# zprodev/zlib.es

Hardware: AMD Instinct MI355X
Metric: GiB/s deflate+inflate round trip, 64 MiB buffers (uncompressed bytes / wall), bit-exact vs reference (higher is better)
Workload: dtype u8; 1 GPU; random64: 1 x 64 MiB xorshift buffer(s) per GPU (seed 12345+index), deflate then inflate, HBM-resident; bytes_per_buffer=67108864, compressed_bytes=67176156, parallelism=independent buffers, one per GPU

## Files before the change

### zlib.es_amd/csrc/zes_inflate_par.hip

```cpp
#include "zes_common.h"
#include "zes_kernels.h"
#include "zes_chain.h"

#define PL_ROOT 10u
#define PD_ROOT 9u
#define F_EOB 1u
#define F_FAIL 2u
#define F_VOID 4u
#define F_HIST 8u

#define RES_W 4096u
#define P4_SPARSE_DEP_MAX 32u
#define P4_SPARSE_MAX 1024u
#ifndef RES_REPS
#define RES_REPS 4u
#endif
#define PAR_CHUNK (ZES_BLK - 3u * RES_W)
#define PAR_DIST_OFF (PAR_CHUNK + 64u)
#define PAR_MAX_OUT (1u << 27)
#define STAGE_DW ((ZES_BLK + ZES_BLK / 8) / 4)
struct ParSmem {
  uint8_t out[ZES_BLK];
  uint32_t bitmap[ZES_BLK / 32];
  uint32_t lut_l[1u << PL_ROOT];
  uint32_t lut_d[1u << PD_ROOT];
  uint8_t len_l[1u << PL_ROOT];
  uint8_t len_d[1u << PD_ROOT];
  uint16_t syms_l[288];
  uint16_t syms_d[32];
  uint32_t first_l[16], first_d[16];
  uint16_t cnt_l[16], cnt_d[16], offs_l[16], offs_d[16];
  uint8_t lens[352];
  uint8_t cl_lut[128];
  uint32_t wave_sum[PAR_WAVES];
  uint8_t wtab[PAR_WAVES][48];
  uint8_t gtab[PAR_WAVES][4][48];
  uint8_t wentry[PAR_WAVES];
  uint32_t hdr_end, status, tail_entry, bfinal, tail_bytes, tail_end;
  uint32_t h_hlit, h_total, h_wbase, h_off, h_k, h_prev, h_done;
  uint32_t res_flag[3];
  uint32_t res_lastw[RES_W / 32];
  uint32_t res_strad[4];
  uint32_t f8lo, f8n, f8off;
  uint32_t sp_n;
};

static_assert(offsetof(ParSmem, cl_lut) - offsetof(ParSmem, lut_l) >= RES_W * 2u, "P4's distance array lies over the decode tables");
static_assert(RES_W % PAR_THREADS == 0 && RES_W % 8u == 0, "P4 lane mapping");

__device__ __forceinline__ static uint32_t entry_l(uint32_t sym, uint32_t len) {
  if (sym < 256u) return len | (sym << 16);
  if (sym == 256u) return len | (1u << 8);
  if (sym < 286u) return len | ((uint32_t)kLenXbits[sym - 257u] << 4) | (2u << 8) | ((uint32_t)kLenBase[sym - 257u] << 16);
  return len | (3u << 8);
}
__device__ __forceinline__ static uint32_t entry_d(uint32_t sym, uint32_t len) {
  if (sym < 30u) return len | ((uint32_t)kDistXbits[sym] << 4) | (2u << 8) | ((uint32_t)kDistBase[sym] << 16);
  return len | (3u << 8);
}

struct BitSrc {
  const uint32_t* g32;
  uint32_t lastdw;
  const uint32_t* s32;
  uint32_t s_first;
  uint32_t s_count;
};
template <bool LDS>
__device__ __forceinline__ static uint32_t src_ldw(const BitSrc& s, uint32_t idx) {
  if (LDS) {
    const uint32_t k = idx - s.s_first;
    return k < s.s_count ? s.s32[k ^ ((k >> 5) & 31u)] : 0u;
  }
  return s.g32[idx < s.lastdw ? idx : s.lastdw];
}

struct LaneBits {
  uint64_t bb;
  uint32_t nb;
  uint32_t pos;
  uint32_t pre;
};
template <bool LDS>
__device__ __forceinline__ static void lb_seek(LaneBits& b, const BitSrc& s, uint32_t bit) {
  const uint32_t i = bit >> 5, sh = bit & 31u;
  const uint64_t w = (uint64_t)src_ldw<LDS>(s, i) | ((uint64_t)src_ldw<LDS>(s, i + 1) << 32);
  b.bb = w >> sh;
  b.nb = 64u - sh;
  b.pos = bit;
  b.pre = LDS ? 0u : src_ldw<LDS>(s, i + 2);
}
template <bool LDS>
__device__ __forceinline__ static void lb_refill(LaneBits& b, const BitSrc& s) {
  if (b.nb <= 32u) {
    if (LDS) {
      b.bb |= (uint64_t)src_ldw<LDS>(s, (b.pos + b.nb) >> 5) << b.nb;
      b.nb += 32u;
    } else {
      b.bb |= (uint64_t)b.pre << b.nb;
      b.nb += 32u;
      b.pre = src_ldw<LDS>(s, (b.pos + b.nb) >> 5);
    }
  }
}
__device__ __forceinline__ static uint32_t lb_take(LaneBits& b, uint32_t k) {
  const uint32_t v = (uint32_t)b.bb & ((1u << k) - 1u);
  b.bb >>= k;
  b.nb -= k;
  b.pos += k;
  return v;
}

struct Lit8 {
  uint32_t lo, n, off;
};
__device__ __forceinline__ static uint32_t lead_lit8(uint32_t w, const Lit8& f) {
  const uint32_t r = __brev(w);
  const bool a = ((r >> 24) - f.lo) < f.n, b = (((r >> 16) & 255u) - f.lo) < f.n, c = (((r >> 8) & 255u) - f.lo) < f.n,
             d = ((r & 255u) - f.lo) < f.n;
  uint32_t n = d ? 4u : 3u;
  n = c ? n : 2u;
  n = b ? n : 1u;
  n = a ? n : 0u;
  return n;
}

struct SegTab {
  uint64_t a, b, c, d, e, f, g, h;
};
__device__ __forceinline__ static uint32_t tab_get(const SegTab& t, uint32_t o) {
  const uint32_t wi = o >> 3;
  uint64_t a = t.a, b = t.b, c = t.c, d = t.d, e = t.e, f = t.f, g = t.g, h = t.h;
  asm("" : "+v"(a), "+v"(b), "+v"(c), "+v"(d));
  asm("" : "+v"(e), "+v"(f), "+v"(g), "+v"(h));
  uint64_t x = a;
  x = (wi == 1u) ? b : x;
  x = (wi == 2u) ? c : x;
  x = (wi == 3u) ? d : x;
  x = (wi == 4u) ? e : x;
  x = (wi == 5u) ? f : x;
  x = (wi == 6u) ? g : x;
  x = (wi == 7u) ? h : x;
  return (uint32_t)(x >> ((o & 7u) * 8u)) & 0xffu;
}
__device__ __forceinline__ static void tab_set(SegTab& t, uint32_t o, uint32_t code) {
  const uint32_t wi = o >> 3;
  const uint64_t v = (uint64_t)code << ((o & 7u) * 8u);
  t.a |= (wi == 0u) ? v : 0ull;
  t.b |= (wi == 1u) ? v : 0ull;
  t.c |= (wi == 2u) ? v : 0ull;
  t.d |= (wi == 3u) ? v : 0ull;
  t.e |= (wi == 4u) ? v : 0ull;
  t.f |= (wi == 5u) ? v : 0ull;
  t.g |= (wi == 6u) ? v : 0ull;
  t.h |= (wi == 7u) ? v : 0ull;
}
__device__ __forceinline__ static void tab_put(SegTab& t, uint32_t o, uint32_t code, bool doit) {
  const uint32_t wi = o >> 3, sh = (o & 7u) * 8u;
  const uint64_t m = doit ? (0xffull << sh) : 0ull, v = doit ? ((uint64_t)code << sh) : 0ull;
  t.a = (wi == 0u) ? ((t.a & ~m) | v) : t.a;
  t.b = (wi == 1u) ? ((t.b & ~m) | v) : t.b;
  t.c = (wi == 2u) ? ((t.c & ~m) | v) : t.c;
  t.d = (wi == 3u) ? ((t.d & ~m) | v) : t.d;
  t.e = (wi == 4u) ? ((t.e & ~m) | v) : t.e;
  t.f = (wi == 5u) ? ((t.f & ~m) | v) : t.f;
  t.g = (wi == 6u) ? ((t.g & ~m) | v) : t.g;
  t.h = (wi == 7u) ? ((t.h & ~m) | v) : t.h;
}
__device__ __forceinline__ static uint64_t tab_nzmask(const SegTab& t) {
  auto nz8 = [](uint64_t w) -> uint64_t {
    const uint64_t k7 = 0x7f7f7f7f7f7f7f7full;
    const uint64_t y = (((w & k7) + k7) | w) & ~k7;
    return ((y >> 7) * 0x0102040810204080ull) >> 56;
  };
  return nz8(t.a) | (nz8(t.b) << 8) | (nz8(t.c) << 16) | (nz8(t.d) << 24) | (nz8(t.e) << 32) | (nz8(t.f) << 40) | (nz8(t.g) << 48) | (nz8(t.h) << 56);
}
__device__ __forceinline__ static uint64_t bcast64(uint64_t v, uint32_t srclane) {
  const uint32_t lo = (uint32_t)__builtin_amdgcn_readlane((int)(uint32_t)v, (int)srclane);
  const uint32_t hi = (uint32_t)__builtin_amdgcn_readlane((int)(uint32_t)(v >> 32), (int)srclane);
  return (uint64_t)lo | ((uint64_t)hi << 32);
}
__device__ __forceinline__ static SegTab tab_bcast(const SegTab& t, uint32_t srclane) {
  SegTab r;
  r.a = bcast64(t.a, srclane);
  r.b = bcast64(t.b, srclane);
  r.c = bcast64(t.c, srclane);
  r.d = bcast64(t.d, srclane);
  r.e = bcast64(t.e, srclane);
  r.f = bcast64(t.f, srclane);
  r.g = bcast64(t.g, srclane);
  r.h = bcast64(t.h, srclane);
  return r;
}

__device__ __forceinline__ static int slow_sym(const LaneBits& b, uint32_t root, const uint16_t* syms, const uint32_t* first,
                                               const uint16_t* cnt, const uint16_t* offs, uint32_t* len_out) {
  uint32_t code = __brev((uint32_t)b.bb & ((1u << root) - 1u)) >> (32u - root);
  for (uint32_t len = root + 1; len <= 15u; len++) {
    code = (code << 1) | (uint32_t)((b.bb >> (len - 1)) & 1u);
    const uint32_t f = first[len];
    const uint32_t rel = code - f;
    if (code >= f && rel < cnt[len]) {
      *len_out = len;
      return (int)syms[offs[len] + rel];
    }
  }
  return -1;
}

#define T_LIT 0u
#define T_EOB 1u
#define T_MATCH 2u
#define T_FAIL 3u
#define C_EOB 62u
#define C_FAIL 63u
#define C_NONE 255u

template <bool LDS>
__device__ __forceinline__ static uint32_t tok_step(ParSmem& S, LaneBits& b, const BitSrc& src, uint32_t& val, uint32_t& len,
                                                    uint32_t& dist) {
  lb_refill<LDS>(b, src);
  uint32_t e = S.lut_l[(uint32_t)b.bb & ((1u << PL_ROOT) - 1u)];
  if ((e & 15u) == 0u) {
    uint32_t l2 = 0;
    const int sy = slow_sym(b, PL_ROOT, S.syms_l, S.first_l, S.cnt_l, S.offs_l, &l2);
    if (sy < 0) return T_FAIL;
    e = entry_l((uint32_t)sy, l2);
  }
  lb_take(b, e & 15u);
  const uint32_t kind = (e >> 8) & 3u;
  if (kind == 0u) {
    val = e >> 16;
    return T_LIT;
  }
  if (kind == 1u) return T_EOB;
  if (kind == 3u) return T_FAIL;
  lb_refill<LDS>(b, src);
  len = (e >> 16) + lb_take(b, (e >> 4) & 15u);
  lb_refill<LDS>(b, src);
  uint32_t ed = S.lut_d[(uint32_t)b.bb & ((1u << PD_ROOT) - 1u)];
  if ((ed & 15u) == 0u) {
    uint32_t l2 = 0;
    const int sy = slow_sym(b, PD_ROOT, S.syms_d, S.first_d, S.cnt_d, S.offs_d, &l2);
    if (sy < 0) return T_FAIL;
    ed = entry_d((uint32_t)sy, l2);
  }
  lb_take(b, ed & 15u);
  if (((ed >> 8) & 3u) != 2u) return T_FAIL;
  lb_refill<LDS>(b, src);
  dist = (ed >> 16) + lb_take(b, (ed >> 4) & 15u);
  return T_MATCH;
}

__device__ __forceinline__ static uint32_t lut_l_entry(ParSmem& S, uint32_t bits) {
  uint32_t e = S.lut_l[bits & ((1u << PL_ROOT) - 1u)];
  if ((e & 15u) == 0u) {
    LaneBits t;
    t.bb = bits;
    uint32_t l2 = 0;
    const int sy = slow_sym(t, PL_ROOT, S.syms_l, S.first_l, S.cnt_l, S.offs_l, &l2);
    e = sy < 0 ? 0u : entry_l((uint32_t)sy, l2);
  }
  return e;
}
__device__ __forceinline__ static uint32_t lut_d_entry(ParSmem& S, uint32_t bits) {
  uint32_t e = S.lut_d[bits & ((1u << PD_ROOT) - 1u)];
  if ((e & 15u) == 0u) {
    LaneBits t;
    t.bb = bits;
    uint32_t l2 = 0;
    const int sy = slow_sym(t, PD_ROOT, S.syms_d, S.first_d, S.cnt_d, S.offs_d, &l2);
    e = sy < 0 ? 0u : entry_d((uint32_t)sy, l2);
  }
  return e;
}

__device__ __forceinline__ static void lb_refill_bf(LaneBits& b, const BitSrc& s) {
  const bool need = b.nb <= 32u;
  const uint32_t k = ((b.pos + b.nb) >> 5) - s.s_first;
  const bool in = k < s.s_count;
  const uint32_t kk = in ? k : 0u;
  uint32_t w = s.s32[kk ^ ((kk >> 5) & 31u)];
  w = in ? w : 0u;
  const uint32_t sh = need ? b.nb : 0u;
  const uint64_t add = (uint64_t)w << sh;
  b.bb |= need ? add : 0ull;
  b.nb += need ? 32u : 0u;
}

__device__ __forceinline__ static void len_step(ParSmem& S, const BitSrc& src, LaneBits& b, bool act, uint32_t& adv, bool& eob,
                                                bool& bad) {
  lb_refill_bf(b, src);
  const uint32_t a = S.len_l[(uint32_t)b.bb & ((1u << PL_ROOT) - 1u)];
  uint32_t n = a & 63u;
  const bool sp = (a & 0x80u) != 0u;
  bool m = (a & 0x40u) != 0u;
  eob = false;
  bad = false;
  if (__ballot(act && sp)) {
    const uint32_t e = lut_l_entry(S, (uint32_t)b.bb);
    const uint32_t kind = (e >> 8) & 3u;
    if (sp) {
      eob = kind == 1u;
      bad = (kind == 3u) || ((e & 15u) == 0u);
      n = (e & 15u) + ((e >> 4) & 15u);
// ... 804 lines not shown
  uint32_t at = 0, len = 0;
#pragma unroll
  for (uint32_t l = 1; l <= ROOT; l++) {
    const uint32_t r = (msb >> (ROOT - l)) - fst[l];
    if (r < cn[l]) {
      at = ofs[l] + r;
      len = l;
    }
  }
  uint32_t ent = 0, bl = 0x80u;
  if (len) {
    const uint32_t sym = syms[at];
    ent = IS_DIST ? entry_d(sym, len) : entry_l(sym, len);
    const uint32_t kind = (ent >> 8) & 3u;
    bl = (ent & 15u) + ((ent >> 4) & 15u);
    if (IS_DIST) bl = (kind == 2u) ? bl : 0x80u;
    else bl = (kind == 0u) ? bl : (kind == 2u) ? (bl | 0x40u) : 0x80u;
  }
  lut[i] = ent;
  blut[i] = (uint8_t)bl;
}

template <int CTRL, int ROWS>
__device__ __forceinline__ static uint32_t ph_dpp(uint32_t old, uint32_t x) {
  return (uint32_t)__builtin_amdgcn_update_dpp((int)old, (int)x, CTRL, ROWS, 0xf, false);
}
__device__ __forceinline__ static uint32_t ph_scan_add(uint32_t x) {
  x += ph_dpp<0x111, 0xf>(0u, x);
  x += ph_dpp<0x112, 0xf>(0u, x);
  x += ph_dpp<0x114, 0xf>(0u, x);
  x += ph_dpp<0x118, 0xf>(0u, x);
  x += ph_dpp<0x142, 0xa>(0u, x);
  x += ph_dpp<0x143, 0xc>(0u, x);
  return x;
}
__device__ __forceinline__ static uint32_t ph_scan_max(uint32_t x) {
  x = max(x, ph_dpp<0x111, 0xf>(0u, x));
  x = max(x, ph_dpp<0x112, 0xf>(0u, x));
  x = max(x, ph_dpp<0x114, 0xf>(0u, x));
  x = max(x, ph_dpp<0x118, 0xf>(0u, x));
  x = max(x, ph_dpp<0x142, 0xa>(0u, x));
  x = max(x, ph_dpp<0x143, 0xc>(0u, x));
  return x;
}

#define HSTAMP(i)                                                          \
  do {                                                                     \
    if (hdbg && zes_lane() == 0) hdbg[16 + (i)] = (unsigned long long)clock64(); \
  } while (0)
template <bool LDS>
__device__ __forceinline__ static bool par_header_fixed(ParSmem& S, const BitSrc& src, uint32_t limit, uint32_t start, unsigned long long* hdbg) {
  const uint32_t lane = zes_lane();
  HSTAMP(0);
  uint32_t bfinal, HLIT, HDIST, HCLEN;
  {
    const uint32_t i = start >> 5, sh = start & 31u;
    const uint64_t w = (uint64_t)src_ldw<LDS>(src, i) | ((uint64_t)src_ldw<LDS>(src, i + 1u) << 32);
    const uint32_t f = (uint32_t)(w >> sh);
    bfinal = f & 1u;
    if (((f >> 1) & 3u) != 2u) return false;
    HLIT = ((f >> 3) & 31u) + 257u;
    HDIST = ((f >> 8) & 31u) + 1u;
    HCLEN = ((f >> 13) & 15u) + 4u;
  }
  uint32_t mycl;
  {
    const uint32_t bp = start + 17u + 3u * (lane < 19u ? lane : 0u);
    const uint32_t j = bp >> 5, s2 = bp & 31u;
    const uint64_t w = (uint64_t)src_ldw<LDS>(src, j) | ((uint64_t)src_ldw<LDS>(src, j + 1u) << 32);
    const uint32_t v = lane < HCLEN ? ((uint32_t)(w >> s2) & 7u) : 0u;
    constexpr uint64_t inv_lo = 3ull | (17ull << 5) | (15ull << 10) | (13ull << 15) | (11ull << 20) | (9ull << 25) | (7ull << 30) | (5ull << 35) | (4ull << 40) |
                                (6ull << 45) | (8ull << 50) | (10ull << 55);
    constexpr uint64_t inv_hi = 12ull | (14ull << 5) | (16ull << 10) | (18ull << 15) | (0ull << 20) | (1ull << 25) | (2ull << 30);
    const uint32_t from = lane < 12u ? (uint32_t)(inv_lo >> (5u * lane)) & 31u : lane < 19u ? (uint32_t)(inv_hi >> (5u * (lane - 12u))) & 31u : 63u;
    mycl = (uint32_t)__builtin_amdgcn_ds_bpermute((int)(from << 2), (int)v);
    if (lane >= 19u) mycl = 0;
  }
  uint32_t kraft = 0;
  {
    uint32_t code = 0, off = 0, e0 = 0, e1 = 0;
    const uint32_t i0 = __brev(lane) >> 25, i1 = __brev(lane + 64u) >> 25;
    uint8_t* sorted = reinterpret_cast<uint8_t*>(S.wave_sum);
    static_assert(sizeof(S.wave_sum) >= 20, "room for the code-length code's symbols");
    uint32_t fst[8], cn[8], ofs[8];
#pragma unroll
    for (uint32_t l = 1; l <= 7; l++) {
      const bool mine = lane < 19 && mycl == l;
      const uint64_t m = __ballot(mine);
      const uint32_t n = (uint32_t)__popcll(m);
      if (mine) sorted[off + (uint32_t)__popcll(m & zes_lanemask_lt())] = (uint8_t)lane;
      fst[l] = code;
      cn[l] = n;
      ofs[l] = off;
      kraft += n << (7 - l);
      code = (code + n) << 1;
      off += n;
    }
    asm volatile("s_waitcnt lgkmcnt(0)" ::: "memory");
    uint32_t a0 = 0, l0 = 0, a1 = 0, l1 = 0;
#pragma unroll
    for (uint32_t l = 1; l <= 7; l++) {
      const uint32_t r0 = (i0 >> (7u - l)) - fst[l], r1 = (i1 >> (7u - l)) - fst[l];
      if (r0 < cn[l]) {
        a0 = ofs[l] + r0;
        l0 = l;
      }
      if (r1 < cn[l]) {
        a1 = ofs[l] + r1;
        l1 = l;
      }
    }
    e0 = l0 ? (uint32_t)sorted[a0] | (l0 << 5) : 0u;
    e1 = l1 ? (uint32_t)sorted[a1] | (l1 << 5) : 0u;
    if (kraft <= 128u) {
      S.cl_lut[lane] = (uint8_t)e0;
      S.cl_lut[lane + 64u] = (uint8_t)e1;
    }
  }
  if (kraft > 128u) return false;
  for (uint32_t i = lane; i < 352; i += 64) S.lens[i] = 0;
  if (lane == 0) {
    const uint32_t p = start + 17u + 3u * HCLEN;
    S.bfinal = bfinal;
    S.h_hlit = HLIT;
    S.h_total = HLIT + HDIST;
    S.h_wbase = p & ~31u;
    S.h_off = p & 31u;
    S.h_done = 0;
  }
  (void)limit;
  HSTAMP(1);
  return true;
}

template <bool LDS>
__device__ __forceinline__ static void par_header_lens(ParSmem& S, const BitSrc& src, uint32_t limit, unsigned long long* hdbg) {
  const uint32_t lane = zes_lane(), wave = threadIdx.x >> 6;
  constexpr uint32_t LP_NONE = 31u;
  uint32_t* s_tab = S.lut_d;
  uint32_t* s_cl = S.lut_l + wave * 64u;
  static_assert(PAR_WAVES * 32u <= (1u << PD_ROOT) && PAR_WAVES * 64u <= (1u << PL_ROOT), "header scratch lies over the tables");
  const uint32_t HLIT = S.h_hlit, total = S.h_total;
  uint32_t wbase0 = S.h_wbase, off0 = S.h_off, k0 = 0, prev0 = 0;
  for (;;) {
    const uint32_t wb = wbase0 + 64u * wave;
    const uint32_t d = wb >> 5;
    const uint32_t w0 = src_ldw<LDS>(src, d), w1 = src_ldw<LDS>(src, d + 1), w2 = src_ldw<LDS>(src, d + 2);
    const uint64_t lo64 = (uint64_t)w0 | ((uint64_t)w1 << 32), hi64 = (uint64_t)w1 | ((uint64_t)w2 << 32);
    const uint32_t bits = lane < 32u ? (uint32_t)(lo64 >> lane) : (uint32_t)(hi64 >> (lane - 32u));
    const uint32_t e = S.cl_lut[bits & 127u];
    const uint32_t l = e >> 5, sy = e & 31u;
    const uint32_t xb = sy == 16u ? 2u : sy == 17u ? 3u : sy == 18u ? 7u : 0u;
    const uint32_t xv = (bits >> l) & ((1u << xb) - 1u);
    const bool valid = l != 0u && (uint64_t)wb + lane + l + xb <= (uint64_t)limit;
    const uint32_t rep = !valid ? 0u : sy == 16u ? 3u + xv : sy == 17u ? 3u + xv : sy == 18u ? 11u + xv : 1u;
    const uint32_t pk = (valid ? lane + l + xb : 64u) | (rep << 7) | (sy << 15) | ((uint32_t)valid << 20);
    uint32_t t = (pk & 127u) | (rep << 7) | ((uint32_t)!valid << 21) | ((!valid || sy == 16u ? LP_NONE : sy >= 17u ? 0u : sy) << 22);
#pragma unroll
    for (int r = 0; r < 6; r++) {
      const uint32_t J = t & 127u;
      const uint32_t u = (uint32_t)__builtin_amdgcn_ds_bpermute((int)(min(J, 63u) << 2), (int)t);
      if (J < 64u) {
        const uint32_t lpu = (u >> 22) & 31u;
        t = (u & 127u) | ((((t >> 7) & 0x3FFFu) + ((u >> 7) & 0x3FFFu)) << 7) | ((t | u) & (1u << 21)) | ((lpu != LP_NONE ? lpu : (t >> 22) & 31u) << 22);
      }
    }
    if (lane < 32u) s_tab[wave * 32u + lane] = t;
    __syncthreads();
    uint32_t en = off0, k = k0, prev = prev0;
    bool past = false, bad = false;
    for (uint32_t v = 0; v < wave; v++) {
      const uint32_t tt = s_tab[v * 32u + en];
      k += (tt >> 7) & 0x3FFFu;
      if (k >= total) {
        past = true;
        break;
      }
      bad = bad || ((tt >> 21) & 1u);
      const uint32_t lpv = (tt >> 22) & 31u;
      prev = lpv != LP_NONE ? lpv : prev;
      en = (tt & 127u) - 64u;
    }
    if (bad && lane == 0) atomicOr(&S.status, 1u);
    if (!past && !bad) {
      uint64_t m = 0;
      uint32_t cur = en, nsym = 0;
      while (cur < 64u) {
        const uint32_t v = (uint32_t)__builtin_amdgcn_readlane((int)pk, (int)cur);
        m |= 1ull << cur;
        nsym++;
        cur = v & 127u;
      }
      asm volatile("s_waitcnt lgkmcnt(0)" ::: "memory");
      if ((m >> lane) & 1ull) s_cl[(uint32_t)__popcll(m & zes_lanemask_lt())] = pk;
      asm volatile("s_waitcnt lgkmcnt(0)" ::: "memory");
      const uint32_t tc = s_cl[lane];
      const bool on = lane < nsym;
      const uint32_t s1 = on ? (tc >> 15) & 31u : 0u, r1 = on ? (tc >> 7) & 255u : 0u;
      const bool hole = on && !((tc >> 20) & 1u);
      const uint32_t is16 = (uint32_t)(on && !hole && s1 == 16u);
      const uint32_t valraw = s1 >= 16u ? 0u : s1;
      const uint32_t srcl = ph_scan_max((on && !is16) ? lane + 1u : 0u);
      const uint32_t vsrc = (uint32_t)__builtin_amdgcn_ds_bpermute((int)((srcl ? srcl - 1u : 0u) << 2), (int)valraw);
      const uint32_t val = srcl ? vsrc : prev;
      const uint32_t kin = ph_scan_add(r1);
      const uint32_t kk = k + kin - r1;
      const uint64_t endm = __ballot(on && !hole && kk + r1 >= total);
      const uint32_t cut = endm ? (uint32_t)__builtin_ctzll(endm) : nsym - 1u;
      const bool mine = on && lane <= cut;
      const uint64_t badm = __ballot(mine && (hole || (is16 && kk == 0u) || kk + r1 > total));
      if (badm) {
        if (lane == 0) atomicOr(&S.status, 1u);
      } else {
        if (mine && val) {
          for (uint32_t q = 0; q < r1; q++) {
            const uint32_t idx = kk + q;
            S.lens[idx < HLIT ? idx : 288 + (idx - HLIT)] = (uint8_t)val;
          }
        }
        if (endm) {
          const uint32_t nx = (uint32_t)__builtin_amdgcn_readlane((int)(tc & 127u), (int)cut);
          if (lane == 0) {
            S.hdr_end = wb + nx;
            S.h_done = 1;
          }
        } else if (wave == PAR_WAVES - 1u && lane == 0) {
          S.h_off = cur - 64u;
          S.h_k = (uint32_t)__builtin_amdgcn_readlane((int)(kk + r1), (int)cut);
          S.h_prev = (uint32_t)__builtin_amdgcn_readlane((int)val, (int)cut);
        }
      }
    }
    __syncthreads();
    if (S.status || S.h_done) break;
    off0 = S.h_off;
    k0 = S.h_k;
    prev0 = S.h_prev;
    wbase0 += 64u * PAR_WAVES;
    __syncthreads();
  }
  if (wave == 0) HSTAMP(2);
  if (!S.status && S.hdr_end > limit && threadIdx.x == 0) S.status = 1;
}

struct ParItem {
  const uint32_t* g32;
  uint32_t lastdw, limit, start;
  uint32_t de_est, de_est2;
  ZesCandRes* cres;
  ZesCandRes* cres_host;
  uint32_t* start_host;
  uint8_t* dst;
  uint64_t room;
  ZesSegRes* sres;
  uint32_t* sym;
  uint64_t sym_cap;
  uint32_t* sym_all;
  unsigned long long* bump;
  uint64_t bump_base, bump_cap;
  uint64_t* symoff;
  uint32_t* map;
  const uint32_t* cand;
  uint32_t ncand;
  uint32_t* fail_list;
  uint32_t w;
};

template <bool FOREIGN, bool TWO>
__device__ __forceinline__ static void par_body(ParSmem& S, const ParItem& it, unsigned long long* dbg) {
#define STAMP(i)                                                     \
  do {                                                               \
    if (dbg && threadIdx.x == 0) dbg[(size_t)blockIdx.x * ZES_PAR_DBG_ROW + (i)] = (unsigned long long)clock64(); \
  } while (0)
#define PAR_DECLINE(END_BIT, TOTAL)                                   \
  do {                                                                \
    if (threadIdx.x == 0) {                                           \
      if (FOREIGN) {                                                  \
        ZesSegRes r_;                                                 \
        r_.end_bit = 0;                                               \
        r_.out_len = 0;                                               \
        r_.flags = 0;                                                 \
        r_.next = 0;                                                  \
        *it.sres = r_;                                                \
        it.fail_list[1u + atomicAdd(&it.fail_list[0], 1u)] = it.w;    \
      } else {                                                        \
        ZesCandRes r_;                                                \
        r_.end_bit = (END_BIT);                                       \
        r_.out_len = (TOTAL);                                         \
        r_.flags = 0;                                                 \
        *it.cres = r_;                                                \
        if (it.cres_host) {                                           \
          *it.cres_host = r_;                                         \
          *it.start_host = it.start;                                  \
        }                                                             \
      }                                                               \
    }                                                                 \
  } while (0)
  const uint32_t tid = threadIdx.x, lane = tid & 63u, wave = tid >> 6;
  const uint32_t lastdw = it.lastdw, limit = it.limit, start = it.start;
  BitSrc src;
  src.g32 = it.g32;
  src.lastdw = lastdw;
  src.s32 = reinterpret_cast<const uint32_t*>(S.out);
  src.s_first = start >> 5;
  uint32_t ds = 0, seg0 = 0, seglen = 0, base = 0, stop = 0, ecode = 0, tail_code = 0;
  uint32_t plimit = limit;
  Lit8 f8 = {0, 0, 0};
  bool p2_global = false;
  STAMP(0);
  auto stage_and_tables = [&](const uint32_t de_est) __attribute__((always_inline)) -> uint32_t {
    {
      const uint64_t end_bit = min((uint64_t)limit, max((uint64_t)de_est, (uint64_t)start + 4800u) + 1280u);
      const uint32_t end_dw = min(lastdw, (uint32_t)((end_bit + 63u) >> 5));
      src.s_count = end_dw - src.s_first + 1u;
      plimit = (uint32_t)min((uint64_t)limit, ((uint64_t)end_dw + 1u) * 32u);
    }
    const bool use_lds = src.s_count <= STAGE_DW;
    if (tid == 0) S.status = use_lds ? 0u : 1u;
    if (use_lds) {
      uint32_t* st = reinterpret_cast<uint32_t*>(S.out);
      for (uint32_t k = tid; k < src.s_count; k += PAR_THREADS) st[k ^ ((k >> 5) & 31u)] = src.g32[src.s_first + k];
    }
    __syncthreads();
    unsigned long long* hdbg = dbg ? dbg + (size_t)blockIdx.x * ZES_PAR_DBG_ROW : nullptr;
    if (wave == 0 && use_lds) {
      const bool ok = par_header_fixed<true>(S, src, plimit, start, hdbg);
      if (!ok && lane == 0) S.status = 1;
    }
    __syncthreads();
    if (S.status) return 1u;
    par_header_lens<true>(S, src, plimit, hdbg);
    __syncthreads();
    if (S.status) return 1u;
    if (wave < 5u) {
      if (!par_build(S, 0, 288, wave, false, S.syms_l, S.first_l, S.cnt_l, S.offs_l) && lane == 0) atomicOr(&S.status, 1u);
    } else if (wave == 5u) {
      if (!par_build(S, 288, 32, 0, true, S.syms_d, S.first_d, S.cnt_d, S.offs_d) && lane == 0) atomicOr(&S.status, 1u);
    }
    __syncthreads();
    if (wave == 0) HSTAMP(3);
    if (S.status) return 1u;
    static_assert(PAR_THREADS == (1u << PL_ROOT) && PAR_THREADS >= (1u << PD_ROOT), "one thread per root-table entry");
    par_fill<PL_ROOT, false>(tid, S.syms_l, S.first_l, S.cnt_l, S.offs_l, S.lut_l, S.len_l);
    if (tid < (1u << PD_ROOT)) par_fill<PD_ROOT, true>(tid, S.syms_d, S.first_d, S.cnt_d, S.offs_d, S.lut_d, S.len_d);
    __syncthreads();
    if (wave == 0) HSTAMP(4);
    STAMP(1);
    ds = S.hdr_end;
    if (!FOREIGN && TWO) {
      if (wave == 0) {
        LaneBits pb;
        lb_seek<true>(pb, src, ds + lane);
        uint32_t v = 0, len = 0, dist = 0;
        const uint32_t kind = (ds + lane < plimit) ? tok_step<true>(S, pb, src, v, len, dist) : T_FAIL;
        const uint32_t w0 = kind | ((pb.pos - (ds + lane)) << 2) | (len << 8);
        uint32_t cur = 0, made = 0;
        bool hist = false;
        for (uint32_t k = 0; k < 16u && cur < 64u; k++) {
          const uint32_t a = (uint32_t)__builtin_amdgcn_readlane((int)w0, (int)cur);
          const uint32_t d = (uint32_t)__builtin_amdgcn_readlane((int)dist, (int)cur);
          const uint32_t kd = a & 3u;
          if (kd == T_LIT) {
            made++;
          } else if (kd == T_MATCH) {
            if (d > made) {
              hist = true;
              break;
            }
            made += (a >> 8) & 511u;
          } else {
            break;
          }
          cur += (a >> 2) & 63u;
        }
        if (hist && lane == 0) S.status = 1u;
      }
      __syncthreads();
      if (S.status) return 1u;
    }
    f8.lo = S.f8lo;
    f8.n = S.f8n;
    f8.off = S.f8off;
    const uint32_t tab_off = ((src.s_count + 31u) & ~31u) * 4u;
    {
      const uint32_t span = de_est > ds ? de_est - ds : 1u;
      seglen = max(64u, (span + PAR_THREADS - 1) / PAR_THREADS);
    }
    const bool dp = TWO && tab_off + DP_BYTES <= STAGE_DW * 4u && !(f8.n && seglen >= 256u);
    seg0 = ds;
    if (dp) {
      seg0 = ds & ~31u;
      const uint32_t span = de_est > seg0 ? de_est - seg0 : 1u;
      seglen = (max(64u, (span + PAR_THREADS - 1) / PAR_THREADS) + 31u) & ~31u;
    }

    const uint64_t b_me64 = (uint64_t)seg0 + (uint64_t)tid * seglen;
    base = (uint32_t)(b_me64 < 0xFFFFFF00ull ? b_me64 : 0xFFFFFF00ull);
    stop = (uint32_t)((b_me64 + seglen) < 0xFFFFFF00ull ? (b_me64 + seglen) : 0xFFFFFF00ull);
    SegTab tab = {0, 0, 0, 0, 0, 0, 0, 0};
    if (dp) {
      uint8_t* T13 = S.out + tab_off + PAR_THREADS * DP_ROW;
      uint8_t* D12 = T13 + (1u << DP_LROOT);
      dp_build(S, T13, D12);
      __syncthreads();
      seg_table_dp(S, src, plimit, base, seglen, T13, D12, S.out + tab_off + tid * DP_ROW);
    } else {
      seg_table<true, TWO>(S, src, plimit, base, stop, f8, tab, dbg ? dbg + (size_t)blockIdx.x * ZES_PAR_DBG_ROW : nullptr);
    }
    STAMP(2);
    const bool room = dp || tab_off + PAR_THREADS * 52u <= STAGE_DW * 4u;
    const bool over = !room && !FOREIGN;
    const bool lds_tabs = room || over;
    const uint32_t toff = over ? 0u : tab_off;
    p2_global = over;
    const uint32_t tstride = dp ? DP_ROW : 52u;
    const uint8_t* tb = S.out + toff + wave * 64u * tstride;
    if (over) __syncthreads();
    if (dp) {
      __syncthreads();
    } else if (lds_tabs) {
      uint32_t* tw = reinterpret_cast<uint32_t*>(S.out + toff) + tid * 13u;
      tw[0] = (uint32_t)tab.a;
      tw[1] = (uint32_t)(tab.a >> 32);
      tw[2] = (uint32_t)tab.b;
      tw[3] = (uint32_t)(tab.b >> 32);
      tw[4] = (uint32_t)tab.c;
      tw[5] = (uint32_t)(tab.c >> 32);
      tw[6] = (uint32_t)tab.d;
      tw[7] = (uint32_t)(tab.d >> 32);
      tw[8] = (uint32_t)tab.e;
      tw[9] = (uint32_t)(tab.e >> 32);
      tw[10] = (uint32_t)tab.f;
      tw[11] = (uint32_t)(tab.f >> 32);
      __syncthreads();
    }
    {
      uint32_t cur = lane;
      if (lds_tabs) {
        uint8_t* gt = &S.gtab[wave][0][0];
#pragma unroll
        for (uint32_t q = 0; q < 3u; q++) {
          const uint32_t idx = lane + 64u * q, grp = idx / 48u, j = idx - 48u * grp;
          uint32_t c = j;
          for (uint32_t sgm = 0; sgm < 16u; sgm++) {
            const uint32_t v = tb[(16u * grp + sgm) * tstride + (c < 48u ? c : 0u)];
            c = c < 48u ? v : c;
          }
          gt[idx] = (uint8_t)c;
        }
        asm volatile("s_waitcnt lgkmcnt(0)" ::: "memory");
#pragma unroll
        for (uint32_t grp = 0; grp < 4u; grp++) {
          const uint32_t v = gt[48u * grp + (cur < 48u ? cur : 0u)];
          cur = cur < 48u ? v : cur;
        }
      } else {
        for (uint32_t sgm = 0; sgm < 64u; sgm++) {
          const SegTab ws = tab_bcast(tab, sgm);
          if (cur < 48u) cur = tab_get(ws, cur);
        }
      }
      if (lane < 48u) S.wtab[wave][lane] = (uint8_t)cur;
    }
    __syncthreads();
    if (tid == 0) {
      uint32_t e = ds - seg0;
      for (uint32_t k = 0; k < PAR_WAVES; k++) {
        S.wentry[k] = (uint8_t)e;
        if (e < 48u) e = S.wtab[k][e];
      }
      S.tail_entry = e;
    }
    __syncthreads();
    uint32_t e = (uint32_t)__builtin_amdgcn_readfirstlane((int)S.wentry[wave]);
    uint32_t mine = C_FAIL;
    if (lds_tabs) {
      const uint8_t* gt = &S.gtab[wave][0][0];
      const uint32_t grp = lane >> 4, upto = lane & 15u;
      uint32_t eg = e, c = e;
#pragma unroll
      for (uint32_t k = 0; k < 3u; k++) {
        eg = eg < 48u ? (uint32_t)gt[48u * k + eg] : eg;
        c = grp == k + 1u ? eg : c;
      }
      for (uint32_t sgm = 0; sgm < 15u; sgm++) {
        const uint32_t v = tb[(16u * grp + sgm) * tstride + (c < 48u ? c : 0u)];
        c = (sgm < upto && c < 48u) ? v : c;
      }
      mine = c;
    } else {
      for (uint32_t sgm = 0; sgm < 64u; sgm++) {
        if (lane == sgm) mine = e;
        const uint32_t own = e < 48u ? tab_get(tab, e) : e;
        e = (uint32_t)__builtin_amdgcn_readlane((int)own, (int)sgm);
      }
    }
    ecode = mine;
    tail_code = S.tail_entry;
    return 0u;
  };
  uint32_t bad = stage_and_tables(it.de_est);
  if (!bad && (tail_code < 48u || tail_code == C_FAIL) && it.de_est2) {
    __syncthreads();
    bad = stage_and_tables(it.de_est2);
  }
  if (bad) {
    PAR_DECLINE(start, 0u);
    return;
  }
  STAMP(3);

  uint32_t entry = base + ecode, exit_pos = 0, outbytes = 0, flags = 0;
  if (!FOREIGN && p2_global)
    seg_run<false, false, FOREIGN>(S, src, plimit, entry, stop, ecode < 48u, f8, 0, exit_pos, outbytes, flags);
  else
    seg_run<false, true, FOREIGN>(S, src, plimit, entry, stop, ecode < 48u, f8, 0, exit_pos, outbytes, flags);
  STAMP(22);
  if (dbg && threadIdx.x == PAR_THREADS - 64) dbg[(size_t)blockIdx.x * ZES_PAR_DBG_ROW + 23] = (unsigned long long)clock64();
  if (ecode >= 48u) flags = F_VOID;
  if (tid == 0) {
    S.tail_bytes = 0;
    S.tail_end = 0;
  }
  __syncthreads();
  for (uint32_t i = tid; i < ZES_BLK / 32; i += PAR_THREADS) S.bitmap[i] = 0;
  uint32_t tail_start = 0;
  if (tail_code < 48u) {
    const uint64_t last_stop = (uint64_t)seg0 + (uint64_t)PAR_THREADS * seglen;
    tail_start = (uint32_t)(last_stop + tail_code);
    if (tid == 0) {
      uint32_t ex, ob, fl;
      seg_decode<false, false, FOREIGN>(S, src, limit, tail_start, 0xFFFFFF00u, 0, ex, ob, fl);
      S.tail_bytes = ob;
      S.tail_end = ex;
      if (!(fl & F_EOB) || (fl & F_FAIL)) atomicOr(&S.status, 2u);
      else atomicOr(&S.status, 4u);
    }
  } else if (tail_code == C_FAIL) {
    if (tid == 0) atomicOr(&S.status, 2u);
  }
  {
    uint32_t incl = outbytes;
#pragma unroll
    for (int dlt = 1; dlt < 64; dlt <<= 1) {
      const uint32_t t = __shfl_up(incl, dlt);
      if ((int)lane >= dlt) incl += t;
    }
    if (lane == 63) S.wave_sum[wave] = incl;
    const uint64_t eobm = __ballot((flags & F_EOB) && !(flags & F_VOID));
    const uint64_t failm = __ballot((flags & F_FAIL) && !(flags & F_VOID));
    if (failm && lane == 0) atomicOr(&S.status, 2u);
    if (eobm && lane == (uint32_t)__builtin_ctzll(eobm)) {
      atomicOr(&S.status, 4u);
      S.hdr_end = exit_pos;
    }
    __syncthreads();
    uint32_t wbase = 0, total = 0;
#pragma unroll
    for (uint32_t k = 0; k < PAR_WAVES; k++) {
      const uint32_t sm = S.wave_sum[k];
      if (k < wave) wbase += sm;
      total += sm;
    }
    const uint32_t seg_total = total;
    total += S.tail_bytes;
    const uint32_t st = S.status;
    const uint32_t end_bit = (tail_code < 48u) ? S.tail_end : S.hdr_end;
    const bool good = (st & 4u) && !(st & 2u) && total <= (FOREIGN ? PAR_MAX_OUT : ZES_BLK) && (FOREIGN || S.bfinal || total == ZES_BLK);
    if (!good) {
      PAR_DECLINE(end_bit, total);
      return;
    }
    const uint32_t my_off = wbase + incl - outbytes;
    STAMP(4);
    uint32_t* symp = it.sym;
    if (FOREIGN) {
      if ((uint64_t)total > it.sym_cap) {
        if (tid == 0) {
          const unsigned long long o = atomicAdd(it.bump, (unsigned long long)((total + 7u) & ~7u));
          S.sp_n = (o + total <= it.bump_cap) ? (uint32_t)(o >> 3) : 0xFFFFFFFFu;
        }
        __syncthreads();
        const uint32_t o8 = S.sp_n;
        __syncthreads();
        if (o8 == 0xFFFFFFFFu) {
          PAR_DECLINE(end_bit, total);
          return;
        }
        symp = it.sym_all + it.bump_base + (uint64_t)o8 * 4u;
      }
      if (tid == 0) *it.symoff = (uint64_t)(symp - it.sym_all);
    }

    uint32_t clo = 0;
    static_assert(PAR_CHUNK % RES_W == 0 && PAR_DIST_OFF + 2u * RES_W <= ZES_BLK, "T2: the distance array lies behind the chunk");
  next_chunk:
    const uint32_t clen = FOREIGN ? min(PAR_CHUNK, total - clo) : total;
    if (FOREIGN) {
      if (tid < 4u) S.res_strad[tid] = 0u;
      if (clo) {
        for (uint32_t i = tid; i < ZES_BLK / 32; i += PAR_THREADS) S.bitmap[i] = 0;
      }
      __syncthreads();
    }
    uint32_t f2 = 0;
    {
      uint32_t ex2, ob2;
      const Lit8 f8e = (FOREIGN && total > PAR_CHUNK) ? Lit8{0, 0, 0} : f8;
      const bool inchunk = !FOREIGN || (my_off < clo + PAR_CHUNK && my_off + outbytes > clo);
      seg_run<true, false, FOREIGN>(S, src, limit, entry, stop, !(flags & F_VOID) && entry < stop && inchunk, f8e, my_off, ex2, ob2, f2, clo);
    }
    if (tid == 0 && tail_code < 48u) {
      uint32_t ex2, ob2, f3 = 0;
      seg_decode<true, false, FOREIGN>(S, src, limit, tail_start, 0xFFFFFF00u, seg_total, ex2, ob2, f3, clo);
      f2 |= f3;
    }
    if (f2 & F_HIST) atomicOr(&S.status, 8u);
    __syncthreads();
    if (S.status & 8u) {
      PAR_DECLINE(end_bit, total);
      return;
    }

    STAMP(5);
    {
      uint16_t* dist = FOREIGN ? reinterpret_cast<uint16_t*>(S.out + PAR_DIST_OFF) : reinterpret_cast<uint16_t*>(S.lut_l);
      if (tid < 3u) S.res_flag[tid] = 0u;
      if (!FOREIGN && tid < 4u) S.res_strad[tid] = 0u;
      __syncthreads();
      unsigned long long tacc[4] = {0, 0, 0, 0}, tlast = dbg ? clock64() : 0ull, nrounds = 0;
#define P4LAP(i)                                         \
  do {                                                   \
    if (dbg && tid == 0) {                               \
      const unsigned long long now_ = clock64();         \
      tacc[i] += now_ - tlast;                           \
      tlast = now_;                                      \
    }                                                    \
  } while (0)
      bool sparse_done = false;
      uint32_t nstarts = 0;
      if (!FOREIGN) {
        static_assert(sizeof(S.lut_l) >= P4_SPARSE_MAX * 4u && sizeof(S.lut_d) >= P4_SPARSE_MAX, "the lists lie over the dead decode tables");
        uint32_t* sp_list = S.lut_l;
        uint8_t* sp_dep = reinterpret_cast<uint8_t*>(S.lut_d);
        uint32_t bw[ZES_BLK / 32 / PAR_THREADS], cnt4 = 0;
#pragma unroll
        for (uint32_t k = 0; k < ZES_BLK / 32 / PAR_THREADS; k++) {
          bw[k] = S.bitmap[tid * (ZES_BLK / 32 / PAR_THREADS) + k];
          cnt4 += (uint32_t)__popc(bw[k]);
        }
        uint32_t incl = cnt4;
#pragma unroll
        for (int dlt = 1; dlt < 64; dlt <<= 1) {
          const uint32_t t = __shfl_up(incl, dlt);
          if ((int)lane >= dlt) incl += t;
        }
        __syncthreads();
        if (lane == 63) S.wave_sum[wave] = incl;
        __syncthreads();
        uint32_t wbase2 = 0, nm = 0;
#pragma unroll
        for (uint32_t k = 0; k < PAR_WAVES; k++) {
          const uint32_t sm = S.wave_sum[k];
          if (k < wave) wbase2 += sm;
          nm += sm;
        }
        nstarts = nm;
        auto rec_of = [&](uint32_t P, uint32_t& D, uint32_t& L) {
          D = ((uint32_t)S.out[P] | ((uint32_t)S.out[P + 1u] << 8)) + 1u;
          L = (uint32_t)S.out[P + 2u] + 3u;
        };
        if (tid == 0) S.sp_n = 0;
        if (nm <= P4_SPARSE_MAX) {
          uint32_t kk = wbase2 + incl - cnt4;
#pragma unroll
          for (uint32_t k = 0; k < ZES_BLK / 32 / PAR_THREADS; k++) {
            uint32_t w = bw[k];
            while (w) {
              const uint32_t bit = (uint32_t)__builtin_ctz(w);
              w &= w - 1u;
              sp_list[kk++] = 32u * (tid * (ZES_BLK / 32 / PAR_THREADS) + k) + bit;
            }
          }
          __syncthreads();
          if (tid < nm) {
            uint32_t P = sp_list[tid], D, L;
            rec_of(P, D, L);
            const uint32_t a = P - D, b = a + min(D, L);
            const uint32_t from = a > (ZES_MAXMATCH - 1u) ? a - (ZES_MAXMATCH - 1u) : 0u;
            uint32_t lo = 0, hi = nm;
            while (lo < hi) {
              const uint32_t mid = (lo + hi) >> 1;
              if (sp_list[mid] < from) lo = mid + 1u; else hi = mid;
            }
            uint32_t dep = 0;
            for (; lo < nm; lo++) {
              const uint32_t Q = sp_list[lo];
              if (Q >= b) break;
              if (Q + (uint32_t)S.out[Q + 2u] + 3u > a) {
                dep = 1;
                break;
              }
            }
            sp_dep[tid] = (uint8_t)dep;
            if (dep) atomicAdd(&S.sp_n, 1u);
          }
          __syncthreads();
          sparse_done = S.sp_n <= P4_SPARSE_DEP_MAX;
        }
        if (sparse_done) {
          auto copy_match = [&](uint32_t P, uint32_t L, uint32_t D) {
            const uint32_t rcp = (D > 1u && D < L) ? 0xFFFFFFFFu / D + 1u : 0u;
            for (uint32_t j = lane; j < L; j += 64u) {
              const uint32_t q = D >= L ? 0u : (D > 1u ? __umulhi(j, rcp) : j);
              S.out[P + j] = S.out[P - D + (j - q * D)];
            }
          };
          for (uint32_t i = wave; i < nm; i += PAR_WAVES) {
            if (sp_dep[i]) continue;
            uint32_t P = sp_list[i], D, L;
            rec_of(P, D, L);
            copy_match(P, L, D);
          }
          __syncthreads();
          if (wave == 0u) {
            for (uint32_t base = 0; base < nm; base += 64u) {
              uint64_t m = __ballot(base + lane < nm && sp_dep[base + lane] != 0u);
              while (m) {
                const uint32_t i = base + (uint32_t)__builtin_ctzll(m);
                m &= m - 1ull;
                uint32_t P = sp_list[i], D, L;
                rec_of(P, D, L);
                copy_match(P, L, D);
              }
            }
          }
          __syncthreads();
        }
      }
      if (FOREIGN) {
        uint32_t c4 = 0;
        for (uint32_t i = tid; i < (clen + 31u) / 32u; i += PAR_THREADS) c4 += (uint32_t)__popc(S.bitmap[i]);
        if (tid == 0) S.sp_n = 0;
        __syncthreads();
        for (int dlt = 32; dlt >= 1; dlt >>= 1) c4 += (uint32_t)__shfl_xor((int)c4, dlt);
        if (lane == 0 && c4) atomicAdd(&S.sp_n, c4);
        __syncthreads();
        nstarts = S.sp_n;
      }
      const bool scanmode = (uint64_t)nstarts * 48u < clen;
      for (uint32_t ws = 0; ws < (sparse_done ? 0u : clen); ws += RES_W) {
        const uint32_t wlen = min(RES_W, clen - ws);
        if (scanmode) {
          if (tid < RES_W / 32u) {
            const uint32_t w = S.bitmap[(ws >> 5) + tid];
            uint32_t hs = w ? 32u * tid + 32u - (uint32_t)__clz(w) : 0u;
#pragma unroll
            for (int dlt = 1; dlt < 64; dlt <<= 1) {
              const uint32_t t = __shfl_up(hs, dlt);
              if ((int)lane >= dlt) hs = max(hs, t);
            }
            S.res_lastw[tid] = hs;
          }
          __syncthreads();
        }
        P4LAP(0);
        uint32_t d[RES_W / PAR_THREADS];
        if (!scanmode) {
          const uint32_t sEnd = S.res_strad[0], sD = S.res_strad[1];
          const uint32_t* out32 = reinterpret_cast<const uint32_t*>(S.out);
          const uint32_t wlo = ws >> 5;
          uint32_t w0[RES_W / PAR_THREADS], w1[RES_W / PAR_THREADS];
#pragma unroll
          for (uint32_t k = 0; k < RES_W / PAR_THREADS; k++) {
            const uint32_t wi = (ws + tid + k * PAR_THREADS) >> 5;
            w0[k] = S.bitmap[wi];
            w1[k] = S.bitmap[wi > wlo ? wi - 1u : wlo];
          }
#pragma unroll
          for (uint32_t k = 0; k < RES_W / PAR_THREADS; k++) {
            const uint32_t bpos = tid + k * PAR_THREADS, P = ws + bpos, wi = P >> 5;
            uint32_t w = w0[k] & (0xFFFFFFFFu >> (31u - (P & 31u)));
            uint32_t bk = 0;
            if (!w && wi > wlo) {
              w = w1[k];
              bk = 1;
            }
            for (uint32_t stg = 0; stg < 2u && !w && wi >= wlo + 2u + 4u * stg; stg++) {
              const uint32_t hiw = wi - 2u - 4u * stg, a = hiw >= wlo + 3u ? hiw - 3u : wlo;
              uint32_t q[4];
              __builtin_memcpy(q, &S.bitmap[a], 16);
#pragma unroll
              for (int t = 3; t >= 0; t--) {
                if (!w && a + (uint32_t)t <= hiw && q[t]) {
                  w = q[t];
                  bk = wi - (a + (uint32_t)t);
                }
              }
            }
            uint32_t dv = 0, e = 0, dd = 0;
            if (w) {
              const uint32_t s = 32u * (wi - bk) + 31u - (uint32_t)__clz(w);
              const uint32_t lo = out32[s >> 2], hi = out32[(s >> 2) + 1u];
              const uint32_t rec = __builtin_amdgcn_alignbyte(hi, lo, s & 3u);
              const uint32_t D = (rec & 0xffffu) + 1u, L = ((rec >> 16) & 0xffu) + 3u;
              dv = P < s + L ? D : 0u;
              e = s + L;
              dd = D;
            } else {
              dv = P < sEnd ? sD : 0u;
            }
            if (bpos == RES_W - 1u) {
              S.res_strad[2] = e > ws + RES_W ? e : 0u;
              S.res_strad[3] = dd;
            }
            dv = bpos < wlen ? dv : 0u;
            d[k] = dv;
            dist[bpos] = (uint16_t)dv;
          }
// ... 429 lines not shown
```

Before: 45.60 GiB/s.

## Stage bitstream into LDS with 128-bit loads and restage after parked tables

Replaces the scalar dword-at-a-time copy of the compressed bitstream into LDS with a 16-byte vectorized loader that handles whole 32-dword rows. It keeps the XOR swizzle by permuting lanes within each vector and aligns the staging base to a 4-dword boundary. When segment tables had to be parked over the staging area, the region is now re-staged from global memory so the decode loop can always use the LDS-backed bit source instead of the global-memory variant. This costs an extra pair of barriers and a reload in that path, and it relies on the new alignment and swizzle remapping matching the reader's indexing.

```diff
diff --git a/zlib.es_amd/csrc/zes_inflate_par.hip b/zlib.es_amd/csrc/zes_inflate_par.hip
--- a/zlib.es_amd/csrc/zes_inflate_par.hip
+++ b/zlib.es_amd/csrc/zes_inflate_par.hip
@@ -1,6 +1,7 @@
 #include "zes_common.h"
 #include "zes_kernels.h"
 #include "zes_chain.h"
+#include <type_traits>
 
 #define PL_ROOT 10u
 #define PD_ROOT 9u
@@ -1411,11 +1412,31 @@
   src.g32 = it.g32;
   src.lastdw = lastdw;
   src.s32 = reinterpret_cast<const uint32_t*>(S.out);
-  src.s_first = start >> 5;
+  src.s_first = (start >> 5) & ~3u;
   uint32_t ds = 0, seg0 = 0, seglen = 0, base = 0, stop = 0, ecode = 0, tail_code = 0;
   uint32_t plimit = limit;
   Lit8 f8 = {0, 0, 0};
-  bool p2_global = false;
+  bool parked_over = false;
+  auto stage_rows = [&](const uint32_t rows, auto turns) __attribute__((always_inline)) {
+    constexpr uint32_t TURNS = decltype(turns)::value;
+    typedef uint32_t Group __attribute__((ext_vector_type(4)));
+    const Group* g128 = reinterpret_cast<const Group*>(src.g32);
+    Group* st = reinterpret_cast<Group*>(S.out);
+    const uint32_t ngrp = rows * 8u, gfirst = src.s_first >> 2, glast = lastdw >> 2;
+    Group v[TURNS];
+#pragma unroll
+    for (uint32_t t = 0; t < TURNS; t++) {
+      const uint32_t k4 = min(tid + t * PAR_THREADS, ngrp - 1u);
+      v[t] = g128[min(gfirst + k4, glast)];
+    }
+#pragma unroll
+    for (uint32_t t = 0; t < TURNS; t++) {
+      const uint32_t k4 = tid + t * PAR_THREADS, r = (k4 >> 3) & 31u;
+      const Group h = (r & 2u) ? v[t].zwxy : v[t];
+      const Group o = (r & 1u) ? h.yxwz : h;
+      if (k4 < ngrp) st[k4 ^ (r >> 2)] = o;
+    }
+  };
   STAMP(0);
   auto stage_and_tables = [&](const uint32_t de_est) __attribute__((always_inline)) -> uint32_t {
     {
@@ -1426,10 +1447,8 @@
     }
     const bool use_lds = src.s_count <= STAGE_DW;
     if (tid == 0) S.status = use_lds ? 0u : 1u;
-    if (use_lds) {
-      uint32_t* st = reinterpret_cast<uint32_t*>(S.out);
-      for (uint32_t k = tid; k < src.s_count; k += PAR_THREADS) st[k ^ ((k >> 5) & 31u)] = src.g32[src.s_first + k];
-    }
+    static_assert(STAGE_DW % 32u == 0 && STAGE_DW / 4u <= 9u * PAR_THREADS, "the staging area in nine turns of whole rows");
+    if (use_lds) stage_rows((src.s_count + 31u) >> 5, std::integral_constant<uint32_t, 9>());
     __syncthreads();
     unsigned long long* hdbg = dbg ? dbg + (size_t)blockIdx.x * ZES_PAR_DBG_ROW : nullptr;
     if (wave == 0 && use_lds) {
@@ -1521,7 +1540,7 @@
     const bool over = !room && !FOREIGN;
     const bool lds_tabs = room || over;
     const uint32_t toff = over ? 0u : tab_off;
-    p2_global = over;
+    parked_over = over;
     const uint32_t tstride = dp ? DP_ROW : 52u;
     const uint8_t* tb = S.out + toff + wave * 64u * tstride;
     if (over) __syncthreads();
@@ -1620,10 +1639,13 @@
   STAMP(3);
 
   uint32_t entry = base + ecode, exit_pos = 0, outbytes = 0, flags = 0;
-  if (!FOREIGN && p2_global)
-    seg_run<false, false, FOREIGN>(S, src, plimit, entry, stop, ecode < 48u, f8, 0, exit_pos, outbytes, flags);
-  else
-    seg_run<false, true, FOREIGN>(S, src, plimit, entry, stop, ecode < 48u, f8, 0, exit_pos, outbytes, flags);
+  if (!FOREIGN && parked_over) {
+    static_assert((PAR_THREADS * 52u) % 128u == 0 && PAR_THREADS * 52u / 16u <= 4u * PAR_THREADS, "the parked tables cover whole rows: four turns");
+    __syncthreads();
+    stage_rows(min(PAR_THREADS * 52u / 128u, (src.s_count + 31u) >> 5), std::integral_constant<uint32_t, 4>());
+    __syncthreads();
+  }
+  seg_run<false, true, FOREIGN>(S, src, plimit, entry, stop, ecode < 48u, f8, 0, exit_pos, outbytes, flags);
   STAMP(22);
   if (dbg && threadIdx.x == PAR_THREADS - 64) dbg[(size_t)blockIdx.x * ZES_PAR_DBG_ROW + 23] = (unsigned long long)clock64();
   if (ecode >= 48u) flags = F_VOID;
```

Result: no change. 46.06 GiB/s, median of 3 (+1.0%).
